# hamidthri/navbot_ppo

Hardware: AMD Instinct MI355X
Metric: env_steps_per_sec (higher is better)
Workload: dtype f32; 1 GPU; BASELINE configs[1]: 4096 envs/GPU, stage_1 (32 segments), 10 beams, PPO mlp64x2, rollout=512, 50 full-batch epochs, episode cap 500; n_envs_total=4096, n_envs_per_gpu=4096, rollout_len=512, epochs=50, policy=mlp64x2, parallelism=env-shard dp1, update_arith=bf16x3, rollout=persistent kernel (navsim_rollout_mlp64)

## Files before the change

### include/navppo.h

```cpp
#ifndef NAVPPO_H
#define NAVPPO_H

#include <stddef.h>
#include <stdint.h>

#ifdef __cplusplus
extern "C" {
#endif

#define NAVPPO_MLP64_ACTOR_PARAMS_D(d) ((d) * 64 + 64 + 64 * 64 + 64 + 64 + 1 + 64 + 1)
#define NAVPPO_MLP64_CRITIC_PARAMS_D(d) ((d) * 64 + 64 + 64 * 64 + 64 + 64 + 1)
#define NAVPPO_MLP64_ACTOR_PARAMS NAVPPO_MLP64_ACTOR_PARAMS_D(16)
#define NAVPPO_MLP64_CRITIC_PARAMS NAVPPO_MLP64_CRITIC_PARAMS_D(16)
#define NAVPPO_MLP64_MAX_BLOCKS 512

const char* navppo_last_error(void);

size_t navppo_mlp64_workspace_bytes(int32_t obs_dim);

int navppo_mlp64_loss_grad(const float* params_dev, const void* obs_dev, int32_t obs_dim, int32_t obs_f16, const float* act_dev,
                           const float* logp_old_dev, const float* rtg_dev, const float* adv_dev, int64_t n_samples,
                           float var, float clip, float* grad_dev, float* stats_dev, void* workspace_dev, void* stream);

int navppo_mlp64_loss_grad_net(int32_t net, const float* params_dev, const void* obs_dev, int32_t obs_dim, int32_t obs_f16,
                               const float* act_dev, const float* logp_old_dev, const float* rtg_dev, const float* adv_dev,
                               int64_t n_samples, float var, float clip, float* grad_dev, float* stats_dev, void* workspace_dev,
                               void* stream);

int navppo_adam_step(float* params_dev, const float* grad_dev, float* adam_m_dev, float* adam_v_dev, int64_t n, float grad_scale,
                     float lr, float beta1, float beta2, float eps, int32_t step, void* stream);

#define NAVPPO_EPISODE_SUMS_WS_BYTES (256 * 6 * 8)
int navppo_episode_sums(const uint8_t* ended_dev, const uint8_t* arrive_dev, const uint8_t* done_dev, const int32_t* ep_length_dev,
                        const float* ep_return_dev, int64_t n, double* sums_dev, void* workspace_dev, void* stream);

int navppo_mlp64_value(const float* critic_params_dev, const void* obs_dev, int32_t obs_dim, int32_t obs_f16, int64_t n_samples,
                       float* value_dev, void* stream);

int navppo_mlp64_update_epoch(float* params_dev, const void* obs_dev, int32_t obs_dim, int32_t obs_f16, const float* act_dev,
                              const float* logp_old_dev, const float* rtg_dev, const float* adv_dev, int64_t n_samples, float var,
                              float clip, float lr, float beta1, float beta2, float eps, int32_t step, float* adam_m_dev,
                              float* adam_v_dev, float* grad_dev, float* stats_dev, void* workspace_dev, void* stream);

int navppo_mlp64_update_epoch_clipped(float* params_dev, const void* obs_dev, int32_t obs_dim, int32_t obs_f16, const float* act_dev,
                                      const float* logp_old_dev, const float* rtg_dev, const float* adv_dev, int64_t n_samples, float var,
                                      float clip, float lr, float beta1, float beta2, float eps, int32_t step, float* adam_m_dev,
                                      float* adam_v_dev, float* grad_dev, float* stats_dev, void* workspace_dev, float max_norm,
                                      float* clip_stats_dev, void* stream);

int navppo_adam_step_clipped(float* params_dev, float* grad_dev, float* adam_m_dev, float* adam_v_dev, int64_t n, int64_t n_first,
                             float grad_scale, float max_norm, float lr, float beta1, float beta2, float eps, int32_t step,
                             float* clip_stats_dev, void* stream);

size_t navppo_mlp64_bf16x3_prep_bytes(int64_t n_samples, int32_t obs_dim );
int navppo_mlp64_bf16x3_prepare(const void* obs_dev, int32_t obs_dim , int32_t obs_f16, int64_t n_samples, void* prep_dev,
                                void* stream);
int navppo_mlp64_bf16x3_loss_grad(const float* params_dev, const void* prep_dev, int32_t obs_dim, const float* act_dev,
                                  const float* logp_old_dev, const float* rtg_dev, const float* adv_dev, int64_t n_samples, float var, float clip,
                                  float* grad_dev, float* stats_dev, void* workspace_dev, void* stream);
int navppo_mlp64_bf16x3_loss_grad_net(int32_t net, const float* params_dev, const void* prep_dev, int32_t obs_dim, const float* act_dev,
                                      const float* logp_old_dev, const float* rtg_dev, const float* adv_dev, int64_t n_samples, float var,
                                      float clip, float* grad_dev, float* stats_dev, void* workspace_dev, void* stream);
int navppo_mlp64_bf16x3_update_epoch(float* params_dev, const void* prep_dev, int32_t obs_dim, const float* act_dev, const float* logp_old_dev,
                                     const float* rtg_dev, const float* adv_dev, int64_t n_samples, float var, float clip, float lr,
                                     float beta1, float beta2, float eps, int32_t step, float* adam_m_dev, float* adam_v_dev,
                                     float* grad_dev, float* stats_dev, void* workspace_dev, void* stream);

int navppo_mlp64_bf16x3_update_epoch_clipped(float* params_dev, const void* prep_dev, int32_t obs_dim, const float* act_dev,
                                             const float* logp_old_dev, const float* rtg_dev, const float* adv_dev, int64_t n_samples, float var,
                                             float clip, float lr, float beta1, float beta2, float eps, int32_t step, float* adam_m_dev,
                                             float* adam_v_dev, float* grad_dev, float* stats_dev, void* workspace_dev, float max_norm,
                                             float* clip_stats_dev, void* stream);

int navppo_mlp64_act(const float* actor_params_dev, const void* obs_dev, int32_t obs_dim, int32_t obs_f16, const float* noise_dev,
                     int64_t n_envs, const float* var_dev, uint64_t seed, uint64_t env_id_base, const uint32_t* step_base_dev,
                     uint32_t step_offset, float* act_dev, float* logp_dev, float* mean_dev, void* stream);

#define NAVPPO_RESMLP512_ACTOR_PARAMS 50290
#define NAVPPO_RESMLP512_CRITIC_PARAMS 50257

size_t navppo_resmlp512_workspace_bytes(int64_t n_samples);

int navppo_resmlp512_loss_grad(const float* params_dev, const void* obs_dev, int32_t obs_f16, const float* act_dev, const float* logp_old_dev,
                               const float* rtg_dev, const float* adv_dev, int64_t n_samples, float var, float clip,
                               float* grad_dev, float* stats_dev, void* workspace_dev, void* stream);

int navppo_resmlp512_update_epoch(float* params_dev, const void* obs_dev, int32_t obs_f16, const float* act_dev, const float* logp_old_dev,
                                  const float* rtg_dev, const float* adv_dev, int64_t n_samples, float var, float clip, float lr,
                                  float beta1, float beta2, float eps, int32_t step, float* adam_m_dev, float* adam_v_dev,
// ... 20 lines not shown
```

### navbot_ppo_amd/_native.py

```python
import ctypes as C
import os

_HERE = os.path.dirname(os.path.abspath(__file__))
LIB_PATH = os.environ.get("NAVSIM_LIB") or os.path.join(_HERE, "libnavsim.so")

NAVSIM_ABI_VERSION = 6


class NavsimError(RuntimeError):
    pass


class NavsimCfg(C.Structure):
    _fields_ = [
        ("n_envs", C.c_int32),
        ("n_beams", C.c_int32),
        ("max_episode_steps", C.c_int32),
        ("auto_reset", C.c_int32),
        ("respawn_on_arrive", C.c_int32),
        ("obs_f16", C.c_int32),
        ("lidar_below_min", C.c_int32),
        ("lidar_noise_sigma", C.c_float),
        ("seed", C.c_uint64),
        ("env_id_base", C.c_uint64),
# ... 23 lines not shown
    ("navsim_destroy", None, [_vp]),
    ("navsim_set_shape", C.c_int, [_vp, _i32, _i32]),
    ("navsim_get_info", C.c_int, [_vp, C.POINTER(NavsimInfo)]),
    ("navsim_set_map", C.c_int, [_vp, _vp, _i32, _i32, _vp]),
    ("navsim_set_goal_rects", C.c_int, [_vp, _i32, _vp, _i32]),
    ("navsim_set_spawn_sampler", C.c_int, [_vp, _vp, _i32, _vp, _i32, _d, _d, _vp]),
    ("navsim_reset", C.c_int, [_vp, _vp, _vp, _vp]),
    ("navsim_step", C.c_int, [_vp] * 12),
    ("navsim_get_state", C.c_int, [_vp] * 8),
    ("navsim_set_state", C.c_int, [_vp] * 8),
    ("navsim_rtg_scan", C.c_int, [_vp, _vp, _i32, _i32, _d, _vp, _i32, _vp]),
    ("navsim_gae_scan", C.c_int, [_vp, _vp, _vp, _vp, _i32, _i32, _d, _d, _vp, _vp, _i32, _vp]),
    ("navsim_raycast", C.c_int, [_vp, _vp, _vp, _vp]),
    ("navsim_odometry", C.c_int, [_i32, _vp, _vp, _vp, _vp, _vp, _vp]),
    ("navsim_rollout_mlp64", C.c_int, [_vp] * 13 + [C.c_uint64, _vp, _i32, _vp]),
    ("navsim_rollout_resmlp512", C.c_int, [_vp] * 13 + [C.c_uint64, _vp, _i32, _vp]),
    ("navsim_step_seq", C.c_int, [_vp, _vp, _i32] + [_vp] * 9),
    ("navsim_evaluate_mlp64", C.c_int, [_vp, _vp, _vp, _i32, _i32] + [_vp] * 7),
    ("navsim_evaluate_resmlp512", C.c_int, [_vp, _vp, _vp, _i32, _i32] + [_vp] * 7),
    ("navppo_last_error", C.c_char_p, []),
    ("navppo_mlp64_workspace_bytes", C.c_size_t, [_i32]),
    ("navppo_mlp64_loss_grad", C.c_int, [_vp, _vp, _i32, _i32] + [_vp] * 4 + [C.c_int64, C.c_float, C.c_float, _vp, _vp, _vp, _vp]),
    ("navppo_mlp64_loss_grad_net", C.c_int, [_i32, _vp, _vp, _i32, _i32] + [_vp] * 4 + [C.c_int64, C.c_float, C.c_float, _vp, _vp, _vp, _vp]),
    ("navppo_adam_step", C.c_int, [_vp, _vp, _vp, _vp, C.c_int64] + [C.c_float] * 5 + [_i32, _vp]),
    ("navppo_mlp64_value", C.c_int, [_vp, _vp, _i32, _i32, C.c_int64, _vp, _vp]),
    ("navppo_episode_sums", C.c_int, [_vp, _vp, _vp, _vp, _vp, C.c_int64, _vp, _vp, _vp]),
    ("navppo_mlp64_update_epoch", C.c_int, [_vp, _vp, _i32, _i32] + [_vp] * 4 + [C.c_int64] + [C.c_float] * 6 + [_i32] + [_vp] * 6),
    ("navppo_mlp64_update_epoch_clipped", C.c_int,
     [_vp, _vp, _i32, _i32] + [_vp] * 4 + [C.c_int64] + [C.c_float] * 6 + [_i32] + [_vp] * 5 + [C.c_float, _vp, _vp]),
    ("navppo_adam_step_clipped", C.c_int, [_vp, _vp, _vp, _vp, C.c_int64, C.c_int64] + [C.c_float] * 6 + [_i32, _vp, _vp]),
    ("navppo_mlp64_act", C.c_int, [_vp, _vp, _i32, _i32, _vp, C.c_int64, _vp, C.c_uint64, C.c_uint64, _vp, C.c_uint32, _vp, _vp, _vp, _vp]),
    ("navppo_mlp64_bf16x3_prep_bytes", C.c_size_t, [C.c_int64, _i32]),
    ("navppo_mlp64_bf16x3_prepare", C.c_int, [_vp, _i32, _i32, C.c_int64, _vp, _vp]),
    ("navppo_mlp64_bf16x3_loss_grad", C.c_int, [_vp, _vp, _i32] + [_vp] * 4 + [C.c_int64, C.c_float, C.c_float, _vp, _vp, _vp, _vp]),
    ("navppo_mlp64_bf16x3_loss_grad_net", C.c_int, [_i32, _vp, _vp, _i32] + [_vp] * 4 + [C.c_int64, C.c_float, C.c_float, _vp, _vp, _vp, _vp]),
    ("navppo_mlp64_bf16x3_update_epoch", C.c_int, [_vp, _vp, _i32] + [_vp] * 4 + [C.c_int64] + [C.c_float] * 6 + [_i32] + [_vp] * 6),
    ("navppo_mlp64_bf16x3_update_epoch_clipped", C.c_int,
     [_vp, _vp, _i32] + [_vp] * 4 + [C.c_int64] + [C.c_float] * 6 + [_i32] + [_vp] * 5 + [C.c_float, _vp, _vp]),
    ("navppo_resmlp512_workspace_bytes", C.c_size_t, [C.c_int64]),
    ("navppo_resmlp512_loss_grad", C.c_int, [_vp, _vp, _i32] + [_vp] * 4 + [C.c_int64, C.c_float, C.c_float, _vp, _vp, _vp, _vp]),
    ("navppo_resmlp512_update_epoch", C.c_int, [_vp, _vp, _i32] + [_vp] * 4 + [C.c_int64] + [C.c_float] * 6 + [_i32] + [_vp] * 6),
    ("navppo_resmlp512_update_epoch_clipped", C.c_int,
     [_vp, _vp, _i32] + [_vp] * 4 + [C.c_int64] + [C.c_float] * 6 + [_i32] + [_vp] * 5 + [C.c_float, _vp, _vp]),
    ("navppo_resmlp512_value", C.c_int, [_vp, _vp, _i32, C.c_int64, _vp, _vp, _vp]),
    ("navppo_resmlp512_act", C.c_int, [_vp, _vp, _i32, _vp, C.c_int64, _vp, C.c_uint64, C.c_uint64, _vp, C.c_uint32, _vp, _vp, _vp, _vp]),
]

_lib = None


def lib():
    global _lib
    if _lib is None:
        if not os.path.exists(LIB_PATH):
            raise NavsimError(f"{LIB_PATH} not found: run `python -c 'import __graft_entry__ as g; g.build()'` "
                              "(hipcc, gfx950).  There is no CPU implementation to fall back to.")
        import torch
        L = C.CDLL(LIB_PATH)
        for name, res, args in SYMBOLS:
            fn = getattr(L, name)
            fn.restype = res
            fn.argtypes = args
        if L.navsim_version() != NAVSIM_ABI_VERSION:
            raise NavsimError(f"libnavsim ABI {L.navsim_version()} != expected {NAVSIM_ABI_VERSION}")
        _lib = L
    return _lib
# ... 7 lines not shown
```

### navbot_ppo_amd/csrc/ppo_mlp64.hip

```cpp
#include <hip/hip_runtime.h>

#include <hip/hip_fp16.h>

#include <cmath>
#include <cstddef>
#include <cstdint>
#include <string>
#include <type_traits>

#include "navppo.h"
#include "navppo_internal.h"
#include "mlp64_policy.h"
#include "bf16x3.h"

namespace {

using namespace mlp64;
static_assert(P_ACTOR == NAVPPO_MLP64_ACTOR_PARAMS && P_CRITIC == NAVPPO_MLP64_CRITIC_PARAMS, "layout");
static_assert(Layout<42>::P_ACTOR == NAVPPO_MLP64_ACTOR_PARAMS_D(42) && Layout<42>::P_CRITIC == NAVPPO_MLP64_CRITIC_PARAMS_D(42) &&
              Layout<16>::P_ACTOR == NAVPPO_MLP64_ACTOR_PARAMS_D(16), "layout");

typedef float f32x16 __attribute__((ext_vector_type(16)));


// ... 66 lines not shown
            const uint2* xp = reinterpret_cast<const uint2*>(reinterpret_cast<const float*>(obs) + m * IN + KH * lhi);
#pragma unroll
            for (int j = 0; j < KH / 2; ++j) {
                uint2 q = make_uint2(0u, 0u);
                if (KH * lhi + 2 * j < IN) q = xp[j];
                raw[2 * j] = q.x;
                raw[2 * j + 1] = q.y;
            }
        } else {
            const uint32_t* xp = reinterpret_cast<const uint32_t*>(reinterpret_cast<const __half*>(obs) + m * IN + KH * lhi);
#pragma unroll
            for (int j = 0; j < KH / 2; ++j) raw[j] = (KH * lhi + 2 * j < IN) ? xp[j] : 0u;
        }
    }
    __device__ __forceinline__ void get(float (&x)[KH]) const {
#pragma unroll
        for (int j = 0; j < KH; ++j) {
            if constexpr (F16) {
                const uint32_t w = raw[j >> 1];
                x[j] = __half2float(__ushort_as_half((unsigned short)((j & 1) ? (w >> 16) : (w & 0xffffu))));
            } else {
                x[j] = __uint_as_float(raw[j]);
            }
        }
    }
};

template <bool F16>
__device__ __forceinline__ float obs_at(const void* __restrict__ obs, const long long idx) {
    if constexpr (F16) return __half2float(reinterpret_cast<const __half*>(obs)[idx]);
    else return reinterpret_cast<const float*>(obs)[idx];
}

template <bool ACTOR, bool FWD = false, int IN = 16, bool F16 = false>
__device__ __forceinline__ void pass_body(SmemW<IN>& sm, const float* __restrict__ params, const void* __restrict__ obs,
                                          const float* __restrict__ act, const float* __restrict__ logp_old,
                                          const float* __restrict__ rtg, const float* __restrict__ adv,
                                          long long M, float var, float clip, float inv_n,
                                          float* __restrict__ partial, float* __restrict__ stats_partial,
                                          float* __restrict__ grad_zero, float* __restrict__ stats_zero,
                                          float* __restrict__ v_out = nullptr) {
    static_assert(!(FWD && ACTOR), "forward-only pass is the critic's");
    using L = Layout<IN>;
    constexpr int OFF_W1 = L::OFF_W1, OFF_B1 = L::OFF_B1, OFF_W2 = L::OFF_W2, OFF_B2 = L::OFF_B2, OFF_W3 = L::OFF_W3,
                  OFF_B3 = L::OFF_B3, OFF_W4 = L::OFF_W4, OFF_B4 = L::OFF_B4;
    constexpr int P = ACTOR ? L::P_ACTOR : L::P_CRITIC;
    constexpr int INP = Pad<IN>::INP, KH = Pad<IN>::KH, NC = Pad<IN>::NC, LW1 = Pad<IN>::LW1;
    constexpr int NW = Pad<IN>::NW;
    constexpr bool kKeepX = (IN == 16) || NW == 4;
    constexpr int NT = 64 * NW;
    const int tid = threadIdx.x, lane = tid & 63, wave = __builtin_amdgcn_readfirstlane(tid >> 6);
    const int l31 = lane & 31, lhi = lane >> 5, l15 = lane & 15, kk = lane >> 4;

    (void)grad_zero;
    (void)stats_zero;
    if constexpr (INP != IN)
        for (int k = tid; k < H * (INP - IN); k += NT) sm.W1s[(k / (INP - IN)) * LW1 + IN + (k % (INP - IN))] = 0.f;
    for (int k = tid; k < H * IN; k += NT) sm.W1s[(k / IN) * LW1 + (k % IN)] = params[OFF_W1 + k];
    for (int k = tid; k < H * H; k += NT) {
        const float w = params[OFF_W2 + k];
        sm.W2s[(k / H) * LW2 + (k % H)] = w;
        sm.W2Ts[(k % H) * LW2 + (k / H)] = w;
    }
    if (tid < H) {
        sm.b1[tid] = params[OFF_B1 + tid];
        sm.b2[tid] = params[OFF_B2 + tid];
        sm.w3[tid] = params[OFF_W3 + tid];
        sm.w4[tid] = ACTOR ? params[OFF_W4 + tid] : 0.f;
    }
    const float b3 = params[OFF_B3];
    const float b4 = ACTOR ? params[OFF_B4] : 0.f;
    __syncthreads();

    float* const T0 = sm.wv + wave * WAVE_F;
    float* const T1 = T0 + TILE_F;
// ... 6 lines not shown
    const float* const w1row = sm.W1s + l31 * LW1 + KH * lhi;
    const float* const w2row = sm.W2s + l31 * LW2 + 4 * lhi;
    const float* const w2trow = sm.W2Ts + l31 * LW2 + 4 * lhi;

    f32x16 aW2[2][2];
    f32x4 aW1[4][NC];
#pragma unroll
    for (int a = 0; a < 2; ++a)
#pragma unroll
        for (int b = 0; b < 2; ++b) aW2[a][b] = zero16();
#pragma unroll
    for (int u = 0; u < 4; ++u)
#pragma unroll
        for (int c = 0; c < NC; ++c) aW1[u][c] = f32x4{0.f, 0.f, 0.f, 0.f};
    float adb2[2] = {0.f, 0.f}, adw3[2] = {0.f, 0.f}, adw4[2] = {0.f, 0.f}, adb1[4] = {0.f, 0.f, 0.f, 0.f};
    float adb3 = 0.f, adb4 = 0.f, st0 = 0.f, st1 = 0.f, st2 = 0.f, st3 = 0.f;

    const long long n_tiles = (M + 31) / 32;
    const long long gw = (long long)blockIdx.x * NW + wave, stride = (long long)gridDim.x * NW;
    XRow<IN, F16> xpre;
    xpre.zero();
    float pre_a0 = 0.f, pre_a1 = 0.f, pre_lp = 0.f, pre_t = 0.f;
    auto prefetch_tile = [&](long long tile) {
        const long long m = tile * 32 + l31;
        xpre.zero();
        if (m < M) {
            xpre.request(obs, m, lhi);
            if (ACTOR) {
                const float2 a = reinterpret_cast<const float2*>(act)[m];
                pre_a0 = a.x;
                pre_a1 = a.y;
                pre_lp = logp_old[m];
                pre_t = adv[m];
            } else if (!FWD) {
                pre_t = rtg[m];
            }
        }
    };
    if (gw < n_tiles) prefetch_tile(gw);
    for (long long tile = gw; tile < n_tiles; tile += stride) {
        const bool valid = tile * 32 + l31 < M;
        float xr[KH];
        xpre.get(xr);
        const float cur_a0 = pre_a0, cur_a1 = pre_a1, cur_lp = pre_lp, cur_t = pre_t;
        if (kKeepX && tile + stride < n_tiles) prefetch_tile(tile + stride);

        f32x16 c1[2];
        {
#pragma unroll
            for (int t = 0; t < 2; ++t)
#pragma unroll
                for (int g = 0; g < 4; ++g) {
                    const float4 b = lds4(sm.b1 + 32 * t + 8 * g + vec_off);
                    c1[t][4 * g] = b.x; c1[t][4 * g + 1] = b.y; c1[t][4 * g + 2] = b.z; c1[t][4 * g + 3] = b.w;
                }
#pragma unroll
            for (int ch = 0; ch < KH / 8; ++ch) {
                float wa[2][8];
#pragma unroll
                for (int t = 0; t < 2; ++t) {
                    const float4 w0 = lds4(w1row + 32 * t * LW1 + 8 * ch), w1 = lds4(w1row + 32 * t * LW1 + 8 * ch + 4);
                    wa[t][0] = w0.x; wa[t][1] = w0.y; wa[t][2] = w0.z; wa[t][3] = w0.w;
                    wa[t][4] = w1.x; wa[t][5] = w1.y; wa[t][6] = w1.z; wa[t][7] = w1.w;
                }
#pragma unroll
                for (int s = 0; s < 8; ++s) {
                    c1[0] = __builtin_amdgcn_mfma_f32_32x32x2f32(wa[0][s], xr[8 * ch + s], c1[0], 0, 0, 0);
                    c1[1] = __builtin_amdgcn_mfma_f32_32x32x2f32(wa[1][s], xr[8 * ch + s], c1[1], 0, 0, 0);
                }
            }
#pragma unroll
            for (int r = 0; r < 16; ++r) {
                c1[0][r] = relu_bits(c1[0][r]);
                c1[1][r] = relu_bits(c1[1][r]);
                const int o = wr_base + (8 * (r >> 2) + (r & 3)) * LT;
                T0[o] = c1[0][r];
                T1[o] = c1[1][r];
            }
// ... 21 lines not shown
                const float a0[4] = {w0.x, w0.y, w0.z, w0.w}, a1[4] = {w1.x, w1.y, w1.z, w1.w};
#pragma unroll
                for (int j = 0; j < 4; ++j) {
                    c2[0] = __builtin_amdgcn_mfma_f32_32x32x2f32(a0[j], c1[t1][4 * g + j], c2[0], 0, 0, 0);
                    c2[1] = __builtin_amdgcn_mfma_f32_32x32x2f32(a1[j], c1[t1][4 * g + j], c2[1], 0, 0, 0);
                }
            }
        }
#pragma unroll
        for (int r = 0; r < 16; ++r) {
            c2[0][r] = relu_bits(c2[0][r]);
            c2[1][r] = relu_bits(c2[1][r]);
        }

        float g3 = 0.f, g4 = 0.f;
        {
            float z3 = 0.f, z4 = 0.f;
#pragma unroll
            for (int t = 0; t < 2; ++t)
#pragma unroll
                for (int g = 0; g < 4; ++g) {
                    const float4 w = lds4(sm.w3 + 32 * t + 8 * g + vec_off);
                    z3 = fmaf(c2[t][4 * g], w.x, z3); z3 = fmaf(c2[t][4 * g + 1], w.y, z3);
                    z3 = fmaf(c2[t][4 * g + 2], w.z, z3); z3 = fmaf(c2[t][4 * g + 3], w.w, z3);
                    if (ACTOR) {
                        const float4 v = lds4(sm.w4 + 32 * t + 8 * g + vec_off);
                        z4 = fmaf(c2[t][4 * g], v.x, z4); z4 = fmaf(c2[t][4 * g + 1], v.y, z4);
                        z4 = fmaf(c2[t][4 * g + 2], v.z, z4); z4 = fmaf(c2[t][4 * g + 3], v.w, z4);
                    }
                }
            z3 += __shfl_xor(z3, 32, 64);
            if (ACTOR) z4 += __shfl_xor(z4, 32, 64);
            if (FWD) {
                if (valid && lhi == 0) v_out[tile * 32 + l31] = z3 + b3;
                if (!kKeepX && tile + stride < n_tiles) prefetch_tile(tile + stride);
                continue;
            }
            const float own = (lhi == 0) ? 1.f : 0.f;
            if (valid) {
                z3 += b3;
                z4 += b4;
#ifdef MLP64_DEBUG_Z
                if (lhi == 0) {
                    float* const dbg = partial + (size_t)200 * P;
                    dbg[tile * 32 + l31] = z3;
                    if (ACTOR) dbg[M + tile * 32 + l31] = z4;
                }
#endif
                if (ACTOR) {
                    const float mu0 = 1.0f / (1.0f + expf(-z3));
                    const float mu1 = tanhf(z4);
                    const float d0 = cur_a0 - mu0, d1 = cur_a1 - mu1;
                    const float lp = -0.5f * ((d0 * d0 + d1 * d1) / var) - 1.8378770664093453f - logf(var);
                    const float lr = lp - cur_lp;
                    const float ratio = expf(lr);
                    const float A = cur_t;
                    const float s1 = ratio * A;
                    const float rc = fminf(fmaxf(ratio, 1.0f - clip), 1.0f + clip);
                    const float s2 = rc * A;
                    st0 += own * -fminf(s1, s2);
                    st2 += own * ((ratio - 1.0f) - lr);
                    st3 += (fabsf(ratio - 1.0f) > clip) ? own : 0.f;
                    const bool inside = (ratio >= 1.0f - clip) && (ratio <= 1.0f + clip);
                    const float dL_dratio = (inside || s1 < s2) ? -A : 0.f;
                    const float dL_dlp = dL_dratio * ratio * inv_n;
                    g3 = dL_dlp * (d0 / var) * (mu0 * (1.0f - mu0));
                    g4 = dL_dlp * (d1 / var) * (1.0f - mu1 * mu1);
// ... 135 lines not shown
            }
            {
                const float4 d0 = lds4(TD + rd16), d1 = lds4(TD + rd16 + 4);
                const float4 e0 = lds4(TD + 16 * LT + rd16), e1 = lds4(TD + 16 * LT + rd16 + 4);
                const float da[8] = {d0.x, d0.y, d0.z, d0.w, d1.x, d1.y, d1.z, d1.w};
                const float ea[8] = {e0.x, e0.y, e0.z, e0.w, e1.x, e1.y, e1.z, e1.w};
                adb1[2 * t1] += ((d0.x + d0.y) + (d0.z + d0.w)) + ((d1.x + d1.y) + (d1.z + d1.w));
                adb1[2 * t1 + 1] += ((e0.x + e0.y) + (e0.z + e0.w)) + ((e1.x + e1.y) + (e1.z + e1.w));
#pragma unroll
                for (int c = 0; c < NC; ++c) {
                    const int cur = kKeepX ? 0 : ((t1 * NC + c) & 1);
                    if constexpr (kKeepX && NC > 1) {
                        const float4 x0 = lds4(T0 + 16 * c * LT + rd16), x1 = lds4(T0 + 16 * c * LT + rd16 + 4);
                        xb[0][0] = x0.x; xb[0][1] = x0.y; xb[0][2] = x0.z; xb[0][3] = x0.w;
                        xb[0][4] = x1.x; xb[0][5] = x1.y; xb[0][6] = x1.z; xb[0][7] = x1.w;
                    }
                    if constexpr (!kKeepX) {
                        if (t1 * NC + c + 1 < 2 * NC) load_xb((c + 1) % NC, xb[cur ^ 1]);
                        __builtin_amdgcn_sched_barrier(0);
                    }
#pragma unroll
                    for (int s = 0; s < 8; ++s) {
                        aW1[2 * t1][c] = __builtin_amdgcn_mfma_f32_16x16x4f32(da[s], xb[cur][s], aW1[2 * t1][c], 0, 0, 0);
                        aW1[2 * t1 + 1][c] = __builtin_amdgcn_mfma_f32_16x16x4f32(ea[s], xb[cur][s], aW1[2 * t1 + 1][c], 0, 0, 0);
                    }
                    if constexpr (!kKeepX) __builtin_amdgcn_sched_barrier(0);
                }
            }
            wave_lds_fence();
        }
        if (!kKeepX && tile + stride < n_tiles) prefetch_tile(tile + stride);
    }

    if (FWD) return;
    __syncthreads();
    constexpr int RP = (P + 3 + 3) & ~3;
    float* const red_base = (IN == 16) ? sm.wv : sm.W2s;
    static_assert(4 * RP <= (int)(sizeof(sm.wv) / sizeof(float)) + ((IN == 16) ? 0 : 2 * H * LW2 + 4 * H), "reduction rows fit");
    float s3 = adb3, s4 = adb4, sA = ACTOR ? st0 : st1, sB = st2, sC = st3;
#pragma unroll
    for (int o = 32; o >= 1; o >>= 1) {
        s3 += __shfl_xor(s3, o, 64); s4 += __shfl_xor(s4, o, 64);
        sA += __shfl_xor(sA, o, 64); sB += __shfl_xor(sB, o, 64); sC += __shfl_xor(sC, o, 64);
    }
    float hb2[2], hw3[2], hw4[2], qb1[4];
#pragma unroll
    for (int t2 = 0; t2 < 2; ++t2) {
        hb2[t2] = adb2[t2] + __shfl_xor(adb2[t2], 32, 64);
        hw3[t2] = adw3[t2] + __shfl_xor(adw3[t2], 32, 64);
        hw4[t2] = adw4[t2] + __shfl_xor(adw4[t2], 32, 64);
    }
#pragma unroll
    for (int u = 0; u < 4; ++u) {
        float v = adb1[u];
        v += __shfl_xor(v, 16, 64);
        v += __shfl_xor(v, 32, 64);
        qb1[u] = v;
    }
    float* const row = red_base + (wave & 3) * RP;
#pragma unroll
    for (int pass = 0; pass < NW / 4; ++pass) {
        if ((wave >> 2) == pass) {
            const bool add = pass >= 1;
            auto put = [&](int idx, float v) { row[idx] = add ? row[idx] + v : v; };
#pragma unroll
            for (int t2 = 0; t2 < 2; ++t2) {
// ... 13 lines not shown
                for (int c = 0; c < NC; ++c)
#pragma unroll
                    for (int r = 0; r < 4; ++r)
                        if (INP == IN || 16 * c + l15 < IN) put(OFF_W1 + (16 * u + 4 * kk + r) * IN + 16 * c + l15, aW1[u][c][r]);
                if (kk == 0) put(OFF_B1 + 16 * u + l15, qb1[u]);
            }
            if (lane == 0) {
                put(OFF_B3, s3);
                if (ACTOR) put(OFF_B4, s4);
                put(P + 0, sA);
                put(P + 1, sB);
                put(P + 2, sC);
            }
        }
        __syncthreads();
    }
    float* out = partial + (size_t)blockIdx.x * P;
    const float* red = red_base;
    for (int k = tid; k < P; k += NT) out[k] = (red[k] + red[RP + k]) + (red[2 * RP + k] + red[3 * RP + k]);
    if (tid < 3) stats_partial[blockIdx.x * 4 + tid] = (red[P + tid] + red[RP + P + tid]) + (red[2 * RP + P + tid] + red[3 * RP + P + tid]);
}

template <bool ACTOR, bool FWD, int IN, bool F16>
__global__ __launch_bounds__(64 * Pad<IN>::NW) void mlp64_pass_w(const float* __restrict__ params, const void* __restrict__ obs,
                                                          const float* __restrict__ act, const float* __restrict__ logp_old,
                                                          const float* __restrict__ rtg, const float* __restrict__ adv,
                                                          long long M, float var, float clip, float inv_n,
                                                          float* __restrict__ partial, float* __restrict__ stats_partial,
                                                          float* __restrict__ grad_zero, float* __restrict__ stats_zero,
                                                          float* __restrict__ v_out = nullptr) {
    __shared__ __attribute__((aligned(16))) SmemW<IN> sm;
    pass_body<ACTOR, FWD, IN, F16>(sm, params, obs, act, logp_old, rtg, adv, M, var, clip, inv_n, partial, stats_partial, grad_zero,
                                   stats_zero, v_out);
}

template <int IN, bool F16>
__global__ __launch_bounds__(64 * Pad<IN>::NW) void mlp64_pass_both(const float* __restrict__ params, const void* __restrict__ obs,
                                                             const float* __restrict__ act, const float* __restrict__ logp_old,
                                                             const float* __restrict__ rtg, const float* __restrict__ adv,
                                                             long long M, float var, float clip, float inv_n,
                                                             float* __restrict__ partial_a, float* __restrict__ stats_partial_a,
                                                             float* __restrict__ partial_c, float* __restrict__ stats_partial_c,
                                                             float* __restrict__ grad, float* __restrict__ stats) {
    __shared__ __attribute__((aligned(16))) SmemW<IN> sm;
    pass_body<true, false, IN, F16>(sm, params, obs, act, logp_old, rtg, adv, M, var, clip, inv_n, partial_a, stats_partial_a, grad,
                                    stats);
    __syncthreads();
    pass_body<false, false, IN, F16>(sm, params + Layout<IN>::P_ACTOR, obs, act, logp_old, rtg, adv, M, var, clip, inv_n, partial_c,
                                     stats_partial_c, grad + Layout<IN>::P_ACTOR, stats + 4);
}

using namespace bf16x3;
#ifdef X3_EXPERIMENT_NO_MFMA
#define X3_MFMA32(a, b, c) ([&] { asm volatile("" ::"v"(a), "v"(b)); return c; }())
#define X3_MFMA16(a, b, c) ([&] { asm volatile("" ::"v"(a), "v"(b)); return c; }())
#else
#define X3_MFMA32(a, b, c) __builtin_amdgcn_mfma_f32_32x32x16_bf16(a, b, c, 0, 0, 0)
#define X3_MFMA16(a, b, c) __builtin_amdgcn_mfma_f32_16x16x32_bf16(a, b, c, 0, 0, 0)
#endif
__device__ __forceinline__ void mma5_small2(f32x16& acc0, f32x16& acc1, const Pieces& A0, const Pieces& A1, const Pieces& B) {
    acc0 = X3_MFMA32(as_bf(A0.p[2]), as_bf(B.p[0]), acc0);
    acc1 = X3_MFMA32(as_bf(A1.p[2]), as_bf(B.p[0]), acc1);
    acc0 = X3_MFMA32(as_bf(A0.p[1]), as_bf(B.p[1]), acc0);
    acc1 = X3_MFMA32(as_bf(A1.p[1]), as_bf(B.p[1]), acc1);
    acc0 = X3_MFMA32(as_bf(A0.p[0]), as_bf(B.p[2]), acc0);
    acc1 = X3_MFMA32(as_bf(A1.p[0]), as_bf(B.p[2]), acc1);
// ... 958 lines not shown
        g_err = "navppo_adam_step_clipped: max_norm must be > 0 (+inf allowed)";
        return -1;
    }
    hipLaunchKernelGGL(sqnorm2_kernel, dim3(1), dim3(kNormThreads), 0, (hipStream_t)stream, (const float*)grad_dev, (int)n, (int)n_first, grad_scale,
                       clip_stats_dev);
    navppo_launch_clip_adam(params_dev, grad_dev, adam_m_dev, adam_v_dev, (int)n, (int)n_first, grad_scale, max_norm, lr, beta1, beta2, eps, step,
                            clip_stats_dev, 1, 1, 8, clip_stats_dev, stream);
    hipError_t e = hipGetLastError();
    if (e != hipSuccess) {
        g_err = std::string("navppo_adam_step_clipped: ") + hipGetErrorString(e);
        return -2;
    }
    return 0;
}

int navppo_mlp64_value(const float* critic_params_dev, const void* obs_dev, int32_t obs_dim, int32_t obs_f16, int64_t n_samples,
                       float* value_dev, void* stream) {
    if (!critic_params_dev || !obs_dev || !value_dev || n_samples < 1 || (obs_dim != 16 && obs_dim != 42) ||
        !obs_aligned(obs_dev, obs_dim, obs_f16)) {
        g_err = "navppo_mlp64_value: bad argument (obs_dim is 16 or 42; obs 16-byte aligned, 42 columns: 8-byte, float16: 4-byte)";
        return -1;
    }
    const long long wtiles = (n_samples + 31) / 32;
    const long long want = (wtiles + kWWaves - 1) / kWWaves;
    const int blocks = (int)(want < kWMaxBlocks ? want : kWMaxBlocks);
    for_obs(obs_dim, obs_f16, [&](auto in, auto f16) {
        hipLaunchKernelGGL((mlp64_pass_w<false, true, decltype(in)::value, decltype(f16)::value>), dim3(blocks), dim3(64 * Pad<decltype(in)::value>::NW), 0,
                           (hipStream_t)stream, critic_params_dev, obs_dev, nullptr, nullptr, nullptr, nullptr, (long long)n_samples, 1.f,
                           0.f, 0.f, nullptr, nullptr, nullptr, nullptr, value_dev);
    });
    hipError_t e = hipGetLastError();
    if (e != hipSuccess) {
        g_err = std::string("navppo_mlp64_value: ") + hipGetErrorString(e);
        return -2;
    }
    return 0;
}

int navppo_mlp64_update_epoch(float* params_dev, const void* obs_dev, int32_t obs_dim, int32_t obs_f16, const float* act_dev,
                              const float* logp_old_dev, const float* rtg_dev, const float* adv_dev, int64_t n_samples, float var,
                              float clip, float lr, float beta1, float beta2, float eps, int32_t step, float* adam_m_dev,
                              float* adam_v_dev, float* grad_dev, float* stats_dev, void* workspace_dev, void* stream) {
    if (!params_dev || !obs_dev || !act_dev || !logp_old_dev || !rtg_dev || !adv_dev || !grad_dev || !stats_dev ||
        !workspace_dev || !adam_m_dev || !adam_v_dev || n_samples < 1 || !(var > 0.f) || step < 1 || (obs_dim != 16 && obs_dim != 42)) {
        g_err = "navppo_mlp64_update_epoch: bad argument (obs_dim is 16 or 42)";
        return -1;
    }
    if (!obs_aligned(obs_dev, obs_dim, obs_f16) || ((uintptr_t)act_dev & 7)) {
        g_err = "navppo_mlp64_update_epoch: obs must be 16-byte (42 columns: 8-byte, float16: 4-byte) and act 8-byte aligned";
        return -1;
    }
    hipStream_t st = (hipStream_t)stream;
    const PassPlan pl = plan_pass(workspace_dev, n_samples, obs_dim);
    const float bc1 = (float)(1.0 - std::pow((double)beta1, (double)step));
    const float bc2_sqrt = (float)std::sqrt(1.0 - std::pow((double)beta2, (double)step));
    for_obs(obs_dim, obs_f16, [&](auto in, auto f16) {
        hipLaunchKernelGGL((mlp64_pass_both<decltype(in)::value, decltype(f16)::value>), dim3(pl.blocks), dim3(64 * Pad<decltype(in)::value>::NW), 0, st, params_dev,
                           obs_dev, act_dev, logp_old_dev, rtg_dev, adv_dev, (long long)n_samples, var, clip, pl.inv_n, pl.partial,
                           pl.stats_partial, pl.partial_c, pl.stats_partial_c, grad_dev, stats_dev);
    });
    hipLaunchKernelGGL(reduce_adam<true>, dim3((pl.pa + pl.pc + 63) / 64), dim3(64 * kRedGroups), 0, st, pl.partial, pl.stats_partial,
                       pl.partial_c, pl.stats_partial_c, pl.blocks, pl.inv_n, grad_dev, stats_dev, params_dev, adam_m_dev, adam_v_dev, lr,
                       beta1, beta2, eps, bc1, bc2_sqrt, pl.pa, pl.pc, 0, pl.pa + pl.pc, pl.gn, (int)(step & 1));
    hipError_t e = hipGetLastError();
    if (e != hipSuccess) {
        g_err = std::string("navppo_mlp64_update_epoch: ") + hipGetErrorString(e);
// ... 215 lines not shown
```

### navbot_ppo_amd/ppo.py

```python
import dataclasses
import math
import os
import time

import torch
import torch.distributed as dist

from . import nets

LOG_2PI = math.log(2.0 * math.pi)


@dataclasses.dataclass
class PPOConfig:
    rollout_len: int = 512
    max_episode_steps: int = 500
    gamma: float = 0.99
    n_updates_per_iteration: int = 50
    lr: float = 3e-4
    clip: float = 0.2
    policy: str = "resmlp512"
    gae_lambda: float = None
    init_var: float = 0.8
    var_decay: float = 0.995
# ... 184 lines not shown
        if self.fused_resmlp512:
            from ._native import lib
            need = lib().navppo_resmlp512_workspace_bytes(int(n)) // 4 + 4
            if self._ws is None or self._ws.numel() < need:
                self._ws = None
                self._ws = torch.empty(need, dtype=torch.float32, device=self.device)
        return self._ws

    def _obs_args(self, obs):
        import ctypes as C
        ok = (torch.float32, torch.float16)
        if obs.dim() != 2 or obs.shape[1] != self.obs_dim or obs.dtype not in ok or not obs.is_contiguous():
            raise ValueError(f"{self.fused}: observations must be contiguous [n, {self.obs_dim}] rows of {ok}, got "
                             f"{tuple(obs.shape)} {obs.dtype}")
        p = C.c_void_p(obs.data_ptr())
        f16 = int(obs.dtype == torch.float16)
        return (p, self.obs_dim, f16) if self.fused_mlp64 else (p, f16)

    def prepare(self, obs):
        import ctypes as C
        from ._native import lib
        L = lib()
        p, d, f16 = self._obs_args(obs)
        need = L.navppo_mlp64_bf16x3_prep_bytes(int(obs.shape[0]), self.obs_dim)
        if self._prep is None or self._prep.numel() < need:
            self._prep = None
            self._prep = torch.empty(need, dtype=torch.uint8, device=self.device)
        rc = L.navppo_mlp64_bf16x3_prepare(p, d, f16, int(obs.shape[0]), C.c_void_p(self._prep.data_ptr()),
                                           C.c_void_p(torch.cuda.current_stream().cuda_stream))
        if rc != 0:
            raise RuntimeError(f"navppo_mlp64_bf16x3_prepare failed: {L.navppo_last_error().decode()}")
        self._prep_key = (obs.data_ptr(), tuple(obs.shape), obs.dtype, obs._version)

    def invalidate_prepared(self):
        self._prep_key = None

    def _prepared(self, obs):
        import ctypes as C
        if self._prep_key != (obs.data_ptr(), tuple(obs.shape), obs.dtype, obs._version):
            self.prepare(obs)
        return C.c_void_p(self._prep.data_ptr())

    def _fused_loss_grad(self, obs, acts, logp_old, rtg, adv, var, stats=None):
        import ctypes as C
        from ._native import lib
        L = lib()
        ptr = lambda t: C.c_void_p(t.data_ptr())
        for t in (acts, logp_old, rtg, adv):
            assert t.is_contiguous() and t.dtype == torch.float32
        name, oargs = (("navppo_mlp64_bf16x3", (self._prepared(obs), self.obs_dim)) if self.bf16x3 else (self.fused, self._obs_args(obs)))
        rc = getattr(L, name + "_loss_grad")(ptr(self.fp.flat), *oargs, ptr(acts), ptr(logp_old), ptr(rtg), ptr(adv),
                                                   int(obs.shape[0]), float(var), float(self.cfg.clip), ptr(self.fp.grad),
                                                   ptr(self._fstats if stats is None else stats), ptr(self._workspace(obs.shape[0])),
                                                   C.c_void_p(torch.cuda.current_stream().cuda_stream))
        if rc != 0:
            raise RuntimeError(f"{self.fused}_loss_grad failed: {L.navppo_last_error().decode()}")

    def _fused_loss_grad_net(self, net, obs, acts, logp_old, rtg, adv, var, stats):
        import ctypes as C
        from ._native import lib
        L = lib()
        ptr = lambda t: C.c_void_p(t.data_ptr())
        fn, oargs = ((L.navppo_mlp64_bf16x3_loss_grad_net, (self._prepared(obs), self.obs_dim)) if self.bf16x3
                     else (L.navppo_mlp64_loss_grad_net, self._obs_args(obs)))
        rc = fn(int(net), ptr(self.fp.flat), *oargs, ptr(acts), ptr(logp_old), ptr(rtg), ptr(adv),
                                          int(obs.shape[0]), float(var), float(self.cfg.clip), ptr(self.fp.grad), ptr(stats),
# ... 117 lines not shown

    def _clip_and_step(self, ep):
        n_a, cs = self.fp.module_numel[0], self.clip_stats
        oks = []
        with torch.no_grad():
            for k, (lo, hi) in enumerate(((0, n_a), (n_a, self.fp.numel))):
                g = self.fp.grad[lo:hi]
                sq = (g * g).sum()
                ok = torch.isfinite(sq)
                coef = torch.where(ok, torch.clamp(self.max_norm / (sq.sqrt() + 1e-6), max=1.0), torch.zeros_like(sq))
                g.mul_(torch.where(ok, coef, torch.ones_like(coef)))
                cs[ep, k], cs[ep, 2 + k] = sq, coef
                oks.append(ok)
            st = self.opt.state.get(self.fp.proxy, {})
            keys = ("exp_avg", "exp_avg_sq")
            old = [self.fp.flat.clone()] + [st[key].clone() if key in st else torch.zeros_like(self.fp.flat) for key in keys]
        self.opt.step()
        with torch.no_grad():
            st = self.opt.state[self.fp.proxy]
            for k, (lo, hi) in enumerate(((0, n_a), (n_a, self.fp.numel))):
                for cur, was in zip([self.fp.flat] + [st[key] for key in keys], old):
                    cur[lo:hi].copy_(torch.where(oks[k], cur[lo:hi], was[lo:hi]))

    def value(self, obs):
        with torch.no_grad():
            if self.fused and obs.is_contiguous() and obs.data_ptr() % 16 == 0 and obs.dtype in (torch.float32, torch.float16):
                return self._fused_value(obs)
            return self.critic(obs.float()).squeeze(-1)

    def update(self, obs, acts, logp_old, rtg, var, adv_raw=None, V0=None):
        cfg, ctx = self.cfg, self.ctx
        world = ctx.world if ctx is not None else 1
        multi = ctx is not None and ctx.enabled
        with torch.no_grad():
            if V0 is None:
                V0 = self.value(obs)
            adv = normalise_advantages(rtg - V0 if adv_raw is None else adv_raw, ctx)
        n_ep = cfg.n_updates_per_iteration
        flat_before = self.fp.flat.clone()
        a_loss = c_loss = torch.zeros((), device=obs.device)
        acc = torch.zeros(6, device=obs.device)
        fused_gn_sq = None
        net_gn = None
        multi_gn = None
        self.loss_history = torch.zeros((n_ep, 2), device=obs.device)
        var_f = float(var) if self.fused else None
        if not (self.fused and obs.dtype == torch.float16):
            obs = obs.float()
        if self.fused:
            obs, acts, logp_old, rtg, adv = (t.contiguous() for t in (obs, acts, logp_old, rtg, adv))
            if self.bf16x3 and n_ep > 0:
                self.prepare(obs)
            if self._fhist.shape[0] < n_ep:
                self._fhist = torch.zeros((n_ep, 8), dtype=torch.float32, device=self.device)
        clipping = self.max_norm is not None
        if clipping:
            self.clip_stats = torch.zeros((max(n_ep, 1), 4), dtype=torch.float32, device=obs.device)
        self._last_adv = adv
        pipelined = self.fused and multi and self.fused_mlp64 and cfg.overlap_allreduce
        if pipelined:
            pg = self._pipelined_epochs(n_ep, world, obs, acts, logp_old, rtg, adv, var_f)
            if n_ep > 0:
                multi_gn = torch.cat([pg.sqrt().sum(0), pg.sum(1).sqrt().sum().reshape(1)])
        for ep in range(n_ep):
            if self.fused:
                if pipelined:
                    pass
                elif multi:
                    self._fused_loss_grad(obs, acts, logp_old, rtg, adv, var_f, stats=self._fhist[ep])
                    ctx.all_reduce_sum(self.fp.grad)
                    if clipping:
                        self._fused_adam(1.0 / world, cstats=self.clip_stats[ep])
                    else:
                        with torch.no_grad():
                            n_a_ = self.fp.module_numel[0]
                            g3 = torch.stack(torch._foreach_norm([self.fp.grad[:n_a_], self.fp.grad[n_a_:], self.fp.grad])) / world
                            multi_gn = g3 if multi_gn is None else multi_gn + g3
                        self._fused_adam(1.0 / world)
                else:
                    self._fused_epoch(obs, acts, logp_old, rtg, adv, var_f, self._fhist[ep], self.clip_stats[ep] if clipping else None)
                if ep == n_ep - 1:
                    h = self._fhist[:n_ep]
                    self.loss_history = h[:, 0:5:4].clone()
                    hs = h.sum(0)
# ... 510 lines not shown
```

Baseline: 56.17 million env-steps/s.

## Fuse critic value, bf16x3 obs prep, and advantage moments into one pass

At the start of each PPO update, one kernel now runs the critic forward pass, writes the bf16x3 split observation pieces, computes raw advantages, and accumulates first and second moments in double precision. A small kernel reduces the per-block moments and a third kernel normalises the advantages. This replaces a separate value pass, a separate prepare pass and several torch elementwise and reduction ops, so observations are read once and fewer launches are issued. The cost is extra LDS traffic and register pressure in the forward kernel, and a variance formula computed from sums that could differ slightly from the previous one.

Result: no change. 56.66 million env-steps/s, median of 6 (+0.9%).

```diff
diff --git a/include/navppo.h b/include/navppo.h
--- a/include/navppo.h
+++ b/include/navppo.h
@@ -55,6 +55,14 @@
 size_t navppo_mlp64_bf16x3_prep_bytes(int64_t n_samples, int32_t obs_dim );
 int navppo_mlp64_bf16x3_prepare(const void* obs_dev, int32_t obs_dim , int32_t obs_f16, int64_t n_samples, void* prep_dev,
                                 void* stream);
+
+#define NAVPPO_MLP64_BEGIN_WS_BYTES (NAVPPO_MLP64_MAX_BLOCKS * 2 * 8)
+int navppo_mlp64_bf16x3_begin_update(const float* critic_params_dev, const void* obs_dev, int32_t obs_dim, int32_t obs_f16,
+                                     const float* rtg_dev, int64_t n_samples, void* prep_dev, float* value_dev, float* adv_raw_dev,
+                                     double* moments_dev, void* workspace_dev, void* stream);
+
+int navppo_normalise_advantages(const float* adv_raw_dev, const double* moments_dev, int64_t n, float* adv_out_dev, void* stream);
+
 int navppo_mlp64_bf16x3_loss_grad(const float* params_dev, const void* prep_dev, int32_t obs_dim, const float* act_dev,
                                   const float* logp_old_dev, const float* rtg_dev, const float* adv_dev, int64_t n_samples, float var, float clip,
                                   float* grad_dev, float* stats_dev, void* workspace_dev, void* stream);
diff --git a/navbot_ppo_amd/_native.py b/navbot_ppo_amd/_native.py
--- a/navbot_ppo_amd/_native.py
+++ b/navbot_ppo_amd/_native.py
@@ -79,6 +79,8 @@
     ("navppo_mlp64_act", C.c_int, [_vp, _vp, _i32, _i32, _vp, C.c_int64, _vp, C.c_uint64, C.c_uint64, _vp, C.c_uint32, _vp, _vp, _vp, _vp]),
     ("navppo_mlp64_bf16x3_prep_bytes", C.c_size_t, [C.c_int64, _i32]),
     ("navppo_mlp64_bf16x3_prepare", C.c_int, [_vp, _i32, _i32, C.c_int64, _vp, _vp]),
+    ("navppo_mlp64_bf16x3_begin_update", C.c_int, [_vp, _vp, _i32, _i32, _vp, C.c_int64, _vp, _vp, _vp, _vp, _vp, _vp]),
+    ("navppo_normalise_advantages", C.c_int, [_vp, _vp, C.c_int64, _vp, _vp]),
     ("navppo_mlp64_bf16x3_loss_grad", C.c_int, [_vp, _vp, _i32] + [_vp] * 4 + [C.c_int64, C.c_float, C.c_float, _vp, _vp, _vp, _vp]),
     ("navppo_mlp64_bf16x3_loss_grad_net", C.c_int, [_i32, _vp, _vp, _i32] + [_vp] * 4 + [C.c_int64, C.c_float, C.c_float, _vp, _vp, _vp, _vp]),
     ("navppo_mlp64_bf16x3_update_epoch", C.c_int, [_vp, _vp, _i32] + [_vp] * 4 + [C.c_int64] + [C.c_float] * 6 + [_i32] + [_vp] * 6),
diff --git a/navbot_ppo_amd/csrc/ppo_mlp64.hip b/navbot_ppo_amd/csrc/ppo_mlp64.hip
--- a/navbot_ppo_amd/csrc/ppo_mlp64.hip
+++ b/navbot_ppo_amd/csrc/ppo_mlp64.hip
@@ -122,15 +122,24 @@
     else return reinterpret_cast<const float*>(obs)[idx];
 }
 
-template <bool ACTOR, bool FWD = false, int IN = 16, bool F16 = false>
+struct BeginArgs {
+    unsigned char* prep = nullptr;
+    float* adv_raw = nullptr;
+    double* mom_partial = nullptr;
+};
+typedef uint16_t __attribute__((may_alias)) lds_u16;
+typedef uint4 __attribute__((may_alias)) lds_u4;
+
+template <bool ACTOR, bool FWD = false, int IN = 16, bool F16 = false, bool BEGIN = false>
 __device__ __forceinline__ void pass_body(SmemW<IN>& sm, const float* __restrict__ params, const void* __restrict__ obs,
                                           const float* __restrict__ act, const float* __restrict__ logp_old,
                                           const float* __restrict__ rtg, const float* __restrict__ adv,
                                           long long M, float var, float clip, float inv_n,
                                           float* __restrict__ partial, float* __restrict__ stats_partial,
                                           float* __restrict__ grad_zero, float* __restrict__ stats_zero,
-                                          float* __restrict__ v_out = nullptr) {
+                                          float* __restrict__ v_out = nullptr, const BeginArgs bg = BeginArgs{}) {
     static_assert(!(FWD && ACTOR), "forward-only pass is the critic's");
+    static_assert(FWD || !BEGIN, "the opening pass of an update is a forward-only pass");
     using L = Layout<IN>;
     constexpr int OFF_W1 = L::OFF_W1, OFF_B1 = L::OFF_B1, OFF_W2 = L::OFF_W2, OFF_B2 = L::OFF_B2, OFF_W3 = L::OFF_W3,
                   OFF_B3 = L::OFF_B3, OFF_W4 = L::OFF_W4, OFF_B4 = L::OFF_B4;
@@ -203,11 +212,12 @@
                 pre_a1 = a.y;
                 pre_lp = logp_old[m];
                 pre_t = adv[m];
-            } else if (!FWD) {
+            } else if (!FWD || BEGIN) {
                 pre_t = rtg[m];
             }
         }
     };
+    double mom0 = 0.0, mom1 = 0.0;
     if (gw < n_tiles) prefetch_tile(gw);
     for (long long tile = gw; tile < n_tiles; tile += stride) {
         const bool valid = tile * 32 + l31 < M;
@@ -215,6 +225,34 @@
         xpre.get(xr);
         const float cur_a0 = pre_a0, cur_a1 = pre_a1, cur_lp = pre_lp, cur_t = pre_t;
         if (kKeepX && tile + stride < n_tiles) prefetch_tile(tile + stride);
+
+        if constexpr (BEGIN) {
+            static_assert(3 * INP * 32 * 2 <= WAVE_F * 4, "the column pieces fit the wave's tiles");
+            unsigned char* const t = bg.prep + (size_t)tile * (2 * 32 * 3 * INP * 2);
+            lds_u16* const colsT = reinterpret_cast<lds_u16*>(T0);
+#pragma unroll
+            for (int j = 0; j < KH / 8; ++j) {
+                float v[8];
+#pragma unroll
+                for (int e = 0; e < 8; ++e) v[e] = xr[8 * j + e];
+                const bf16x3::Pieces Pc = bf16x3::split8(v);
+                const int f0 = KH * lhi + 8 * j;
+#pragma unroll
+                for (int i = 0; i < 3; ++i) {
+                    *reinterpret_cast<uint4*>(t + ((l31 * 3 + i) * INP + f0) * 2) = Pc.p[i];
+                    const uint32_t w[4] = {Pc.p[i].x, Pc.p[i].y, Pc.p[i].z, Pc.p[i].w};
+#pragma unroll
+                    for (int e = 0; e < 8; ++e)
+                        colsT[(i * INP + f0 + e) * 32 + l31] = (uint16_t)((e & 1) ? (w[e >> 1] >> 16) : (w[e >> 1] & 0xffffu));
+                }
+            }
+            wave_lds_fence();
+            const lds_u4* const src = reinterpret_cast<const lds_u4*>(T0);
+            uint4* const dst = reinterpret_cast<uint4*>(t + 32 * 3 * INP * 2);
+#pragma unroll
+            for (int k = 0; k < 12 * INP / 64; ++k) dst[64 * k + lane] = src[64 * k + lane];
+            wave_lds_fence();
+        }
 
         f32x16 c1[2];
         {
@@ -302,7 +340,16 @@
             z3 += __shfl_xor(z3, 32, 64);
             if (ACTOR) z4 += __shfl_xor(z4, 32, 64);
             if (FWD) {
-                if (valid && lhi == 0) v_out[tile * 32 + l31] = z3 + b3;
+                if (valid && lhi == 0) {
+                    const float v0 = z3 + b3;
+                    v_out[tile * 32 + l31] = v0;
+                    if constexpr (BEGIN) {
+                        const float a = cur_t - v0;
+                        bg.adv_raw[tile * 32 + l31] = a;
+                        mom0 += (double)a;
+                        mom1 += (double)a * (double)a;
+                    }
+                }
                 if (!kKeepX && tile + stride < n_tiles) prefetch_tile(tile + stride);
                 continue;
             }
@@ -504,6 +551,25 @@
         if (!kKeepX && tile + stride < n_tiles) prefetch_tile(tile + stride);
     }
 
+    if constexpr (BEGIN) {
+#pragma unroll
+        for (int o = 32; o >= 1; o >>= 1) {
+            mom0 += __shfl_xor(mom0, o, 64);
+            mom1 += __shfl_xor(mom1, o, 64);
+        }
+        __syncthreads();
+        double* const red = reinterpret_cast<double*>(sm.wv);
+        if (lane == 0) {
+            red[2 * wave] = mom0;
+            red[2 * wave + 1] = mom1;
+        }
+        __syncthreads();
+        if (tid < 2) {
+            double s = 0.0;
+            for (int w = 0; w < NW; ++w) s += red[2 * w + tid];
+            bg.mom_partial[2 * blockIdx.x + tid] = s;
+        }
+    }
     if (FWD) return;
     __syncthreads();
     constexpr int RP = (P + 3 + 3) & ~3;
@@ -583,6 +649,51 @@
     __shared__ __attribute__((aligned(16))) SmemW<IN> sm;
     pass_body<ACTOR, FWD, IN, F16>(sm, params, obs, act, logp_old, rtg, adv, M, var, clip, inv_n, partial, stats_partial, grad_zero,
                                    stats_zero, v_out);
+}
+
+template <int IN, bool F16>
+__global__ __launch_bounds__(64 * Pad<IN>::NW) void mlp64_begin_update(const float* __restrict__ critic_params, const void* __restrict__ obs,
+                                                                const float* __restrict__ rtg, long long M, float* __restrict__ v_out,
+                                                                const BeginArgs bg) {
+    __shared__ __attribute__((aligned(16))) SmemW<IN> sm;
+    pass_body<false, true, IN, F16, true>(sm, critic_params, obs, nullptr, nullptr, rtg, nullptr, M, 1.f, 0.f, 0.f, nullptr, nullptr, nullptr,
+                                          nullptr, v_out, bg);
+}
+
+__global__ __launch_bounds__(kWMaxBlocks) void moments_final(const double* __restrict__ partial, int blocks, double n, double* __restrict__ out) {
+    __shared__ double rows[2][kWMaxBlocks];
+    const int t = threadIdx.x;
+    rows[0][t] = t < blocks ? partial[2 * t] : 0.0;
+    rows[1][t] = t < blocks ? partial[2 * t + 1] : 0.0;
+    __syncthreads();
+    if (t < 2) {
+        double s = 0.0;
+#pragma unroll 16
+        for (int b = 0; b < kWMaxBlocks; ++b) s += rows[t][b];
+        out[t] = s;
+    } else if (t == 2) {
+        out[2] = n;
+    }
+}
+
+constexpr int kNormAdvThreads = 256, kNormAdvQuads = 4;
+__global__ __launch_bounds__(kNormAdvThreads) void normalise_adv_kernel(const float* __restrict__ adv_raw, const double* __restrict__ moments,
+                                                                        long long n, float* __restrict__ out, int vec) {
+    const double m0 = moments[0], m1 = moments[1], cnt = moments[2];
+    const double mean = m0 / cnt;
+    const double var = (m1 - cnt * mean * mean) / (cnt - 1.0);
+    const double sd = sqrt(var < 0.0 ? 0.0 : var);
+    const float mean_f = (float)mean, den = (float)sd + 1e-10f;
+#pragma unroll
+    for (int j = 0; j < kNormAdvQuads; ++j) {
+        const long long q = ((long long)blockIdx.x * kNormAdvQuads + j) * kNormAdvThreads + threadIdx.x;
+        if (vec && 4 * q + 3 < n) {
+            const float4 a = reinterpret_cast<const float4*>(adv_raw)[q];
+            reinterpret_cast<float4*>(out)[q] = make_float4((a.x - mean_f) / den, (a.y - mean_f) / den, (a.z - mean_f) / den, (a.w - mean_f) / den);
+        } else {
+            for (long long k = 4 * q; k < n && k < 4 * q + 4; ++k) out[k] = (adv_raw[k] - mean_f) / den;
+        }
+    }
 }
 
 template <int IN, bool F16>
@@ -1607,6 +1718,55 @@
     hipError_t e = hipGetLastError();
     if (e != hipSuccess) {
         g_err = std::string("navppo_mlp64_value: ") + hipGetErrorString(e);
+        return -2;
+    }
+    return 0;
+}
+
+int navppo_mlp64_bf16x3_begin_update(const float* critic_params_dev, const void* obs_dev, int32_t obs_dim, int32_t obs_f16,
+                                     const float* rtg_dev, int64_t n_samples, void* prep_dev, float* value_dev, float* adv_raw_dev,
+                                     double* moments_dev, void* workspace_dev, void* stream) {
+    if (!critic_params_dev || !obs_dev || !rtg_dev || !prep_dev || !value_dev || !adv_raw_dev || !moments_dev || !workspace_dev ||
+        n_samples < 1 || (obs_dim != 16 && obs_dim != 42) || !obs_aligned(obs_dev, obs_dim, obs_f16) || ((uintptr_t)prep_dev & 15) ||
+        ((uintptr_t)moments_dev & 7) || ((uintptr_t)workspace_dev & 7)) {
+        g_err = "navppo_mlp64_bf16x3_begin_update: bad argument (obs_dim is 16 or 42; obs aligned as for navppo_mlp64_value, prep 16-byte, "
+                "moments and workspace 8-byte aligned)";
+        return -1;
+    }
+    const long long wtiles = (n_samples + 31) / 32;
+    const long long want = (wtiles + kWWaves - 1) / kWWaves;
+    const int blocks = (int)(want < kWMaxBlocks ? want : kWMaxBlocks);
+    BeginArgs bg;
+    bg.prep = reinterpret_cast<unsigned char*>(prep_dev);
+    bg.adv_raw = adv_raw_dev;
+    bg.mom_partial = reinterpret_cast<double*>(workspace_dev);
+    static_assert(2 * kWMaxBlocks * sizeof(double) <= NAVPPO_MLP64_BEGIN_WS_BYTES, "moment partials fit the documented scratch");
+    for_obs(obs_dim, obs_f16, [&](auto in, auto f16) {
+        hipLaunchKernelGGL((mlp64_begin_update<decltype(in)::value, decltype(f16)::value>), dim3(blocks), dim3(64 * Pad<decltype(in)::value>::NW), 0,
+                           (hipStream_t)stream, critic_params_dev, obs_dev, rtg_dev, (long long)n_samples, value_dev, bg);
+    });
+    hipLaunchKernelGGL(moments_final, dim3(1), dim3(kWMaxBlocks), 0, (hipStream_t)stream, (const double*)bg.mom_partial, blocks, (double)n_samples,
+                       moments_dev);
+    hipError_t e = hipGetLastError();
+    if (e != hipSuccess) {
+        g_err = std::string("navppo_mlp64_bf16x3_begin_update: ") + hipGetErrorString(e);
+        return -2;
+    }
+    return 0;
+}
+
+int navppo_normalise_advantages(const float* adv_raw_dev, const double* moments_dev, int64_t n, float* adv_out_dev, void* stream) {
+    if (!adv_raw_dev || !moments_dev || !adv_out_dev || n < 1 || ((uintptr_t)moments_dev & 7)) {
+        g_err = "navppo_normalise_advantages: bad argument (moments 8-byte aligned)";
+        return -1;
+    }
+    const int vec = !(((uintptr_t)adv_raw_dev | (uintptr_t)adv_out_dev) & 15);
+    const long long quads = (n + 3) / 4, per_block = (long long)kNormAdvThreads * kNormAdvQuads;
+    hipLaunchKernelGGL(normalise_adv_kernel, dim3((unsigned)((quads + per_block - 1) / per_block)), dim3(kNormAdvThreads), 0,
+                       (hipStream_t)stream, adv_raw_dev, moments_dev, (long long)n, adv_out_dev, vec);
+    hipError_t e = hipGetLastError();
+    if (e != hipSuccess) {
+        g_err = std::string("navppo_normalise_advantages: ") + hipGetErrorString(e);
         return -2;
     }
     return 0;
diff --git a/navbot_ppo_amd/ppo.py b/navbot_ppo_amd/ppo.py
--- a/navbot_ppo_amd/ppo.py
+++ b/navbot_ppo_amd/ppo.py
@@ -240,6 +240,42 @@
             raise RuntimeError(f"navppo_mlp64_bf16x3_prepare failed: {L.navppo_last_error().decode()}")
         self._prep_key = (obs.data_ptr(), tuple(obs.shape), obs.dtype, obs._version)
 
+    def begin_update(self, obs, rtg):
+        import ctypes as C
+        from ._native import lib
+        L = lib()
+        p, d, f16 = self._obs_args(obs)
+        n = int(obs.shape[0])
+        assert rtg.is_contiguous() and rtg.dtype == torch.float32 and rtg.numel() == n
+        need = L.navppo_mlp64_bf16x3_prep_bytes(n, self.obs_dim)
+        if self._prep is None or self._prep.numel() < need:
+            self._prep = None
+            self._prep = torch.empty(need, dtype=torch.uint8, device=self.device)
+        V0 = torch.empty(n, dtype=torch.float32, device=self.device)
+        adv_raw = torch.empty(n, dtype=torch.float32, device=self.device)
+        moments = torch.empty(3, dtype=torch.float64, device=self.device)
+        self._prep_key = None
+        ptr = lambda t: C.c_void_p(t.data_ptr())
+        rc = L.navppo_mlp64_bf16x3_begin_update(C.c_void_p(self.fp.flat.data_ptr() + 4 * self._n_actor), p, d, f16, ptr(rtg), n,
+                                                ptr(self._prep), ptr(V0), ptr(adv_raw), ptr(moments), ptr(self._workspace(n)),
+                                                C.c_void_p(torch.cuda.current_stream().cuda_stream))
+        if rc != 0:
+            raise RuntimeError(f"navppo_mlp64_bf16x3_begin_update failed: {L.navppo_last_error().decode()}")
+        self._prep_key = (obs.data_ptr(), tuple(obs.shape), obs.dtype, obs._version)
+        return V0, adv_raw, moments
+
+    def normalise(self, adv_raw, moments):
+        import ctypes as C
+        from ._native import lib
+        L = lib()
+        assert adv_raw.is_contiguous() and adv_raw.dtype == torch.float32 and moments.dtype == torch.float64 and moments.numel() == 3
+        out = torch.empty_like(adv_raw)
+        rc = L.navppo_normalise_advantages(C.c_void_p(adv_raw.data_ptr()), C.c_void_p(moments.data_ptr()), int(adv_raw.numel()),
+                                           C.c_void_p(out.data_ptr()), C.c_void_p(torch.cuda.current_stream().cuda_stream))
+        if rc != 0:
+            raise RuntimeError(f"navppo_normalise_advantages failed: {L.navppo_last_error().decode()}")
+        return out
+
     def invalidate_prepared(self):
         self._prep_key = None
 
@@ -423,11 +459,20 @@
         cfg, ctx = self.cfg, self.ctx
         world = ctx.world if ctx is not None else 1
         multi = ctx is not None and ctx.enabled
+        n_ep = cfg.n_updates_per_iteration
+        fused_front = (self.bf16x3 and adv_raw is None and V0 is None and obs.dim() == 2 and obs.shape[0] > 0 and obs.shape[1] == self.obs_dim
+                       and obs.dtype in (torch.float32, torch.float16) and obs.is_contiguous() and obs.data_ptr() % 16 == 0
+                       and rtg.dtype == torch.float32)
         with torch.no_grad():
-            if V0 is None:
-                V0 = self.value(obs)
-            adv = normalise_advantages(rtg - V0 if adv_raw is None else adv_raw, ctx)
-        n_ep = cfg.n_updates_per_iteration
+            if fused_front:
+                V0, a_raw, moments = self.begin_update(obs, rtg.contiguous())
+                if ctx is not None:
+                    ctx.all_reduce_sum(moments)
+                adv = self.normalise(a_raw, moments)
+            else:
+                if V0 is None:
+                    V0 = self.value(obs)
+                adv = normalise_advantages(rtg - V0 if adv_raw is None else adv_raw, ctx)
         flat_before = self.fp.flat.clone()
         a_loss = c_loss = torch.zeros((), device=obs.device)
         acc = torch.zeros(6, device=obs.device)
@@ -440,7 +485,7 @@
             obs = obs.float()
         if self.fused:
             obs, acts, logp_old, rtg, adv = (t.contiguous() for t in (obs, acts, logp_old, rtg, adv))
-            if self.bf16x3 and n_ep > 0:
+            if self.bf16x3 and n_ep > 0 and not fused_front:
                 self.prepare(obs)
             if self._fhist.shape[0] < n_ep:
                 self._fhist = torch.zeros((n_ep, 8), dtype=torch.float32, device=self.device)
```
